# kocurvik/mdrp

Measured on AMD Instinct MI355X. Metric: image-pairs/sec (2000 corrs, 10k RANSAC iters), higher is better.
Workload: dtype f64

## Files before the change

### mdrp_amd/csrc/mdrp_capi.hip

```cpp
#include "../../include/mdrp.h"
#include "mdrp_kernels.h"
#include "mdrp_classic.h"
#include "mdrp_frontend.h"
#include "mdrp_schedule.h"
#include "mdrp_from_model.h"
#ifdef MDRP_SPLIT_TU
#define MDRP_INST extern
#include "mdrp_instances.h"
namespace mdrp {
MDRP_INSTANCES_FINAL_64
MDRP_INSTANCES_FINAL_256
MDRP_INSTANCES_CLASSIC
MDRP_INSTANCES_FROM_MODEL
}
#endif

#include <algorithm>
#include <cmath>
#include <cstdio>
#include <cstdlib>
#include <cstddef>
#include <cstring>
#include <functional>
#include <map>
// ... 483 lines not shown
        v.model_count = h->model_count[odd].as<int32_t>() + 2 * q; v.und_count = h->und_count.as<int32_t>() + 2 * q;
        v.surv1 = h->surv_count.as<int32_t>() + q; v.surv2 = h->surv2_count.as<int32_t>() + q;
        v.cand_stat = h->cand_stat.as<unsigned long long>() + 2 * q;
        v.rfrag = h->rfrag.as<uint4>() + q * groups_max * 64; v.trig = h->triggers.as<Trigger>() + q * trig_cap;
        return v;
    }

    int solve(const ChunkView &v, hipStream_t st_) {
        const RunParams &r = v.r;
        const int pc = v.pc;
        HIPCHK(hipMemsetAsync(v.model_count, 0, sizeof(int32_t) * 2 * pc, st_));
        if (v.c < 2 && presampled[v.c]) HIPCHK(hipStreamWaitEvent(st_, h->ev_sampled[v.c], 0));
        else samples(st_, r.chunk_len, v.samples);
        hipEvent_t v0, v1;
        if (int rc = get_events(h, &v0, &v1, 5)) return rc;
        HIPCHK(hipEventRecord(v0, st_));
        struct Stop { hipEvent_t e; hipStream_t s; ~Stop() { (void)hipEventRecord(e, s); } } stop_{v1, st_};
        if (classic) {
            const dim3 sgrid((r.chunk_len + 63) / 64, pc);
            if (kind == MDRP_SHARED_6PT)
                hipLaunchKernelGGL(kc_solve<CLASSIC_SHARED>, sgrid, dim3(64), 0, st_, r, v.st, v.samples, v.pts, v.models, v.slot_inl, v.tags, v.model_count);
            else if (kind == MDRP_RELPOSE_5PT) {
                const bool first_region = v.c == 0 && lay.n_chunks > 1;
                if (first_region && (size_t)sgrid.x > sz.red5_first_blocks) { g_err = "5-point first chunk longer than its Reduce5 region"; return MDRP_ERR_INVALID; }
                double *red5 = h->red5.as<double>() + ((first_region ? (size_t)batch * sz.red5_blocks : 0) + (size_t)v.p0 * sgrid.x) * RED5_STRIDE * 64;
                hipLaunchKernelGGL(kc_solve5_null, sgrid, dim3(64), SOLVE5N_LDS_BYTES, st_, r, v.st, v.samples, v.pts, red5);
                hipLaunchKernelGGL(kc_solve5_reduce, sgrid, dim3(64), SOLVE5_LDS_BYTES, st_, r, v.st, red5);
                hipLaunchKernelGGL(kc_solve5_roots, sgrid, dim3(64), SOLVE5B_LDS_BYTES, st_, r, v.st, v.samples, v.pts, red5, v.models, v.slot_inl, v.tags, v.model_count);
            }
            else
                hipLaunchKernelGGL(kc_solve<CLASSIC_FUND>, sgrid, dim3(64), SOLVE7_LDS_BYTES, st_, r, v.st, v.samples, v.pts, v.models, v.slot_inl, v.tags, v.model_count);
            return MDRP_OK;
        }
#define MDRP_SOLVE_LAUNCH(S)                                                                                                   \
    hipLaunchKernelGGL(k_solve<S>, dim3((r.chunk_len + solve_threads(S) - 1) / solve_threads(S), pc), dim3(solve_threads(S)), 0, st_, r, v.st, v.samples, v.pts, v.dep, v.models, v.slot_inl, v.tags, v.model_count, 0, r.chunk_len)
        switch (r.solver) {
        case SOLVER_P3P: MDRP_SOLVE_LAUNCH(SOLVER_P3P); break;
        case SOLVER_SHIFT: MDRP_SOLVE_LAUNCH(SOLVER_SHIFT); break;
        case SOLVER_SHARED: MDRP_SOLVE_LAUNCH(SOLVER_SHARED); break;
        default: MDRP_SOLVE_LAUNCH(SOLVER_VARYING); break;
        }
#undef MDRP_SOLVE_LAUNCH
        return MDRP_OK;
    }

    int count(const ChunkView &v) {
        unsigned long long *cstats = &cnt->progress.evals;
        hipEvent_t c0, c1;
        if (int rc = get_events(h, &c0, &c1, 1)) return rc;
        const bool two_phase = !v.first_of_run;
        uint32_t *tags_u = v.tags_sorted;
        int32_t *und_part = reinterpret_cast<int32_t *>(v.tags_sorted_other), *cplan = h->cplan.as<int32_t>();
        hipLaunchKernelGGL(k_count_plan, dim3(1), dim3(PLAN_THREADS), 0, s, v.pc, v.st, v.model_count, 2, CNT_WG_MODELS, cplan,
                           v.surv1, (const int32_t *)nullptr, two_phase ? v.und_count : (int32_t *)nullptr);
        const dim3 cgrid((unsigned)v.pc * (unsigned)((v.r.chunk_len * mps + CNT_WG_MODELS - 1) / CNT_WG_MODELS));
        HIPCHK(hipEventRecord(c0, s));
        MDRP_SWEEP_DISPATCH(k_count, kind, cgrid, dim3(CNT_THREADS), 0, s, v.r, v.st, v.rfrag, v.models,
                            v.tags, v.model_count, cplan, v.tags_v, v.surv1, cstats, (int32_t *)nullptr, (const int32_t *)nullptr,
                            1, tags_u, und_part, v.und_count, (const int32_t *)nullptr, v.cand_stat);
        if (two_phase) {
            hipLaunchKernelGGL(k_count_plan, dim3(1), dim3(PLAN_THREADS), 0, s, v.pc, v.st, v.und_count, 2, CNT_WG_MODELS, cplan,
                               (int32_t *)nullptr, (const int32_t *)nullptr, (int32_t *)nullptr);
            MDRP_SWEEP_DISPATCH(k_count, kind, cgrid, dim3(CNT_THREADS), 0, s, v.r, v.st, v.rfrag, v.models,
                                tags_u, v.und_count, cplan, v.tags_v, v.surv1, cstats, (int32_t *)nullptr, (const int32_t *)nullptr,
                                2, (uint32_t *)nullptr, (int32_t *)nullptr, (int32_t *)nullptr, und_part, v.cand_stat);
            h->count_launches++;
        }
        HIPCHK(hipEventRecord(c1, s));
        h->count_launches++;
        return MDRP_OK;
    }

    int bound(const ChunkView &v, Survivors &sv) {
        sv = Survivors{v.tags_v, v.surv1};
        if (!(use_bound && batch_call > 16 && !v.first_of_run)) return MDRP_OK;
        hipLaunchKernelGGL(k_count_plan, dim3(1), dim3(PLAN_THREADS), 0, s, v.pc, v.st, v.surv1, 1, BND_THREADS, h->cplan.as<int32_t>(), v.surv2, (const int32_t *)nullptr);
        const dim3 bgrid((unsigned)v.pc * (unsigned)((v.r.chunk_len * mps + BND_THREADS - 1) / BND_THREADS));
        unsigned long long *bstats = &cnt->progress.evals_bound;
        hipEvent_t b0, b1;
        if (int rc = get_events(h, &b0, &b1, 4)) return rc;
        HIPCHK(hipEventRecord(b0, s));
        MDRP_SWEEP_DISPATCH(k_bound, kind, bgrid, dim3(BND_THREADS), 0, s, v.r, v.st, v.pts, v.models, v.tags_v, v.surv1, h->cplan.as<int32_t>(), v.tags, v.surv2, bstats);
        HIPCHK(hipEventRecord(b1, s));
        sv = Survivors{v.tags, v.surv2};
        return MDRP_OK;
    }

    int score(const ChunkView &v, const Survivors &sv, hipEvent_t e0, hipEvent_t e1) {
        const bool wave = batch_call <= SCORE_WAVE_MAX_PAIRS, split = !wave && score_split && !v.first_of_run;
        const int models = v.r.chunk_len * mps;
        int32_t *plan = h->plan.as<int32_t>(), *totals = plan + 2 * (size_t)batch + 2;
        if (wave) hipLaunchKernelGGL(k_count_plan, dim3(1), dim3(PLAN_THREADS), 0, s, v.pc, v.st, sv.count, 1, SCW_THREADS / 64, plan, (int32_t *)nullptr, (const int32_t *)nullptr, (int32_t *)nullptr);
        hipLaunchKernelGGL(k_sort_tags, dim3(v.pc), dim3(256), 0, s, v.r, v.st, v.model_count, sv.count, sv.tags, v.tags_sorted);
        if (!wave) hipLaunchKernelGGL(k_plan, dim3(1), dim3(PLAN_THREADS), 0, s, v.pc, v.model_count, plan, totals, split ? SPLIT_HYP : SCORE_THREADS);
        HIPCHK(hipEventRecord(e0, s));
        const long long capped = (long long)h->num_cu * 32;
        if (wave) {
            const long long ub = (long long)v.pc * ((models + SCW_THREADS / 64 - 1) / (SCW_THREADS / 64));
            MDRP_SWEEP_DISPATCH(k_score_w, kind, dim3((unsigned)std::min(ub, capped)), dim3(SCW_THREADS), 0, s, v.r, v.st, v.pts, v.models, v.tags_sorted, v.model_count,
                                v.slot_score, v.slot_inl, plan);
        } else if (split) {
            const long long ub = (long long)v.pc * ((models + SPLIT_HYP - 1) / SPLIT_HYP + 1);
            MDRP_SWEEP_DISPATCH(k_score_split, kind, dim3((unsigned)std::min(ub, capped)), dim3(SPLIT_THREADS), 0, s, v.r, v.st, v.pts, v.models, v.tags_sorted, v.model_count,
                                v.slot_score, v.slot_inl, plan, totals);
        } else {
            const dim3 grid((unsigned)v.pc * (unsigned)((models + SCORE_THREADS - 1) / SCORE_THREADS));
            MDRP_SWEEP_DISPATCH(k_score, kind, grid, dim3(SCORE_THREADS), SCORE_TILE_BYTES, s, v.r, v.st, v.pts, v.models, v.tags_sorted, v.model_count,
                                v.slot_score, v.slot_inl, plan, totals);
        }
        HIPCHK(hipEventRecord(e1, s));
        h->sweep_launches++;
        return MDRP_OK;
    }

    void scan(const ChunkView &v) {
        unsigned long long *scan_stats = &cnt->progress.evals_sweep;
#define MDRP_SCAN(M, I) hipLaunchKernelGGL((k_scan<M, I>), dim3(v.pc), dim3(64), 0, s, v.r, v.st, v.slot_score, v.slot_inl, v.trig, trig_cap, v.model_count, scan_stats)
        if (mps == 16) MDRP_SCAN(16, 1);
// ... 1046 lines not shown
```

### mdrp_amd/csrc/mdrp_kernels.h

```cpp
#pragma once
#include <hip/hip_runtime.h>
#include <float.h>
#include "mdrp_logtab.h"
#include "mdrp_math.h"

#ifdef MDRP_SECONDARY_TU
#define MDRP_GLOBAL static __global__
#else
#define MDRP_GLOBAL __global__
#endif

namespace mdrp {

constexpr int PT_STRIDE = 6;
#define MDRP_TILE_PTS 512
#define MDRP_SCORE_MINWAVES 4
constexpr int TILE_PTS = MDRP_TILE_PTS;
constexpr size_t SCORE_TILE_BYTES = (size_t)TILE_PTS * (PT_STRIDE * sizeof(double) + 4 * sizeof(float));
#define MDRP_P1F_UNROLL 8
constexpr int PRUNE_EVERY = 4;
#define MDRP_DENSE_KEY 40
#define MDRP_SOLVE_MINWAVES 2
#define MDRP_SCORE_THREADS 256
constexpr int SCORE_THREADS = MDRP_SCORE_THREADS;
// ... 637 lines not shown
        const int mid = (lo + hi) >> 1;
        if (prefix[mid] <= w) lo = mid; else hi = mid;
    }
    return lo;
}

struct SweepItem { int pair; bool dense, live; uint32_t slot; size_t slot_base; };
__device__ __forceinline__ SweepItem sweep_item(const RunParams &rp, const int32_t *__restrict__ plan, const int32_t *__restrict__ model_count,
                                                const uint32_t *__restrict__ tags, int w, int per_wg, int idx) {
    SweepItem it;
    it.pair = plan_find(plan, rp.batch, w);
    const int blk_sparse = plan[rp.batch + 1 + it.pair];
    const int bi = w - plan[it.pair];
    it.dense = bi >= blk_sparse;
    const int i = (it.dense ? bi - blk_sparse : bi) * per_wg + idx;
    it.slot_base = (size_t)it.pair * rp.slot_stride;
    const int cnt_sparse = model_count[2 * it.pair], cnt_dense = model_count[2 * it.pair + 1];
    it.live = i < (it.dense ? cnt_dense : cnt_sparse);
    it.slot = it.live ? tags[it.slot_base + (it.dense ? rp.slot_stride - 1 - i : i)] : 0;
    return it;
}

#define MDRP_CNT_TILES 8
constexpr int CNT_TILES = MDRP_CNT_TILES;
constexpr int CNT_ROUNDS = (16 * CNT_TILES) / 64;
static_assert(CNT_TILES == 4 || CNT_TILES == 8, "a wavefront owns 64 or 128 hypotheses");
constexpr int CNT_WAVE_MODELS = 16 * CNT_TILES;
constexpr int CNT_THREADS = 256;
constexpr int CNT_WG_MODELS = CNT_WAVE_MODELS * (CNT_THREADS / 64);
typedef __bf16 bf16x8_t __attribute__((ext_vector_type(8)));
typedef float f32x4_t __attribute__((ext_vector_type(4)));

constexpr int PLAN_THREADS = 1024;
__device__ __forceinline__ int plan_block_scan(int v, int &total, int *s_w) {
    const int lane = threadIdx.x & 63, wave = threadIdx.x >> 6;
    int inc = v;
#pragma unroll
    for (int o = 1; o < 64; o <<= 1) { const int u = __shfl_up(inc, o, 64); if (lane >= o) inc += u; }
    __syncthreads();
    if (lane == 63) s_w[wave] = inc;
    __syncthreads();
    if (wave == 0) {
        const int x = lane < PLAN_THREADS / 64 ? s_w[lane] : 0;
        int xi = x;
#pragma unroll
        for (int o = 1; o < PLAN_THREADS / 64; o <<= 1) { const int u = __shfl_up(xi, o, 64); if (lane >= o) xi += u; }
        if (lane < PLAN_THREADS / 64) s_w[lane] = xi - x;
        if (lane == PLAN_THREADS / 64 - 1) s_w[PLAN_THREADS / 64] = xi;
    }
    __syncthreads();
    total = s_w[PLAN_THREADS / 64];
    return inc - v + s_w[wave];
}
MDRP_GLOBAL __launch_bounds__(PLAN_THREADS) void k_count_plan(int batch, const PairState *__restrict__ st, const int32_t *__restrict__ counts, int stride,
                                                             int per_wg, int32_t *__restrict__ plan, int32_t *__restrict__ zero_a,
                                                             const int32_t *__restrict__ begin = nullptr, int32_t *__restrict__ zero_b2 = nullptr ) {
    __shared__ int s_w[PLAN_THREADS / 64 + 1];
    int run = 0;
    for (int p0 = 0; p0 < batch; p0 += PLAN_THREADS) {
        const int p = p0 + threadIdx.x;
        const int b = (p < batch && st[p].active) ? (counts[stride * p] - (begin ? begin[stride * p] : 0) + per_wg - 1) / per_wg : 0;
        int tot;
        const int ex = plan_block_scan(b, tot, s_w);
        if (p < batch) { plan[p] = run + ex; if (zero_a) zero_a[p] = 0; if (zero_b2) zero_b2[2 * p] = 0; }
        run += tot;
    }
    if (threadIdx.x == 0) plan[batch] = run;
}

__device__ __forceinline__ int count_split_tiles(const PairState &ps, int n_tiles, const unsigned long long *__restrict__ cand_stat, int pair) {
    if (!(ps.best_min_score < DBL_MAX) || n_tiles < 4 || !cand_stat) return n_tiles;
    const unsigned long long cs = cand_stat[2 * pair], es = cand_stat[2 * pair + 1];
    if (es == 0) return n_tiles;
    const double rec_score = ps.best_min_score * (1.0 + 1e-12);
    long long bar = (long long)floor((double)ps.n - rec_score / ps.sq_thr);
    if (bar > (long long)ps.best_min_cnt) bar = (long long)ps.best_min_cnt;
    if (bar <= 0) return n_tiles;
    const double g = fmin(0.5, 1.1 * (double)cs / (double)es + 0.005);
    const long long ra = (long long)((double)((long long)ps.n - bar) / (1.0 - g)) + 32;
    const int ta = (int)((ra + 255) >> 8);
    return ta + 2 > n_tiles ? n_tiles : ta;
}

template <bool POSE, bool RAWF = false>
__global__ __launch_bounds__(CNT_THREADS, 4) void k_count(RunParams rp, const PairState *__restrict__ st, const uint4 *__restrict__ rfrag,
                                                          const Model *__restrict__ models, const uint32_t *__restrict__ tags,
                                                          const int32_t *__restrict__ model_count, const int32_t *__restrict__ plan,
                                                          uint32_t *__restrict__ tags_surv,
                                                          int32_t *__restrict__ surv_count, unsigned long long *__restrict__ stats,
                                                          int32_t *__restrict__ cand_out ,
                                                          const int32_t *__restrict__ tag_begin = nullptr ,
                                                          int phase = 0, uint32_t *__restrict__ tags_und = nullptr, int32_t *__restrict__ und_part = nullptr,
                                                          int32_t *__restrict__ und_count = nullptr, const int32_t *__restrict__ part_in = nullptr,
                                                          unsigned long long *__restrict__ cand_stat = nullptr ) {
    constexpr int A_TILE_GROUPS = 16;
    __shared__ uint4 s_lds[2 * A_TILE_GROUPS * 64];
    uint4 (*s_frag)[CNT_WAVE_MODELS][4] = reinterpret_cast<uint4 (*)[CNT_WAVE_MODELS][4]>(s_lds);
    static_assert(sizeof(uint4) * (CNT_THREADS / 64) * CNT_WAVE_MODELS * 4 <= sizeof(uint4) * 2 * A_TILE_GROUPS * 64, "fragment staging fits the tile buffers");
    const int total = plan[rp.batch];
    const int w = blockIdx.x;
    if (w >= total) return;
    const int pair = plan_find(plan, rp.batch, w);
    const int blk = w - plan[pair];
    const PairState &ps = st[pair];
    const int tbeg = tag_begin ? tag_begin[2 * pair] : 0;
    const int n = ps.n, cnt = model_count[2 * pair] - tbeg;
    const int tid = threadIdx.x, lane = tid & 63, wave = tid >> 6;
    const int m0 = blk * CNT_WG_MODELS + wave * CNT_WAVE_MODELS;
    const size_t slot_base = (size_t)pair * rp.slot_stride;
    const uint32_t *tags_p = tags + slot_base + tbeg;
    const double thr = ps.sq_thr;
    uint32_t slot_r[CNT_ROUNDS] = {};
    int part_r[CNT_ROUNDS] = {};
    Model mr[CNT_ROUNDS];
#pragma unroll
    for (int r = 0; r < CNT_ROUNDS; ++r) {
        const int i = m0 + 64 * r + lane;
        if (i < cnt) { slot_r[r] = tags_p[i] & 0xFFFFFFu; if (phase == 2) part_r[r] = part_in[slot_base + tbeg + i]; }
    }
#pragma unroll
    for (int r = 0; r < CNT_ROUNDS; ++r) {
        const Model *mp = models + slot_base + slot_r[r];
        const double2 *P = reinterpret_cast<const double2 *>(mp);
        const double2 q01 = P[0], q23 = P[1], t01 = P[2], t2s = P[3], f12 = P[5];
        mr[r].q[0] = q01.x; mr[r].q[1] = q01.y; mr[r].q[2] = q23.x; mr[r].q[3] = q23.y;
        mr[r].t[0] = t01.x; mr[r].t[1] = t01.y; mr[r].t[2] = t2s.x;
        mr[r].f1 = f12.x; mr[r].f2 = f12.y;
        mr[r].scale = t2s.y; mr[r].shift1 = RAWF ? P[4].x : 0.0;
    }
#pragma unroll
    for (int r = 0; r < CNT_ROUNDS; ++r) {
        const int i = m0 + 64 * r + lane;
        uint16_t eh[8], el[8], e8[3];
        float tb = 1.0f;
#pragma unroll
        for (int j = 0; j < 8; ++j) { eh[j] = 0; el[j] = 0; }
        e8[0] = e8[1] = e8[2] = 0;
        if (i < cnt) {
            double E[9];
            model_matrix<POSE, RAWF>(mr[r], E);
            count_setup_scaled(E, ps.box, thr, eh, el, e8, tb);
        }
        uint4 *dst = s_frag[wave][64 * r + lane];
        dst[0] = pack_bf16x8(eh);
        dst[1] = pack_bf16x8(el);
        dst[2] = make_uint4((uint32_t)e8[0] | ((uint32_t)e8[1] << 16), (uint32_t)e8[2], 0u, 0u);
        dst[3] = make_uint4(__float_as_uint(tb), 0u, 0u, 0u);
    }
    __syncthreads();
    const bool idle = m0 >= cnt;
    const int col = lane & 15, ksl = lane >> 4;
    const int part = ksl < 2 ? 0 : ksl - 1;
    bf16x8_t bfrag[CNT_TILES];
    float tbv[CNT_TILES];
    float cand[CNT_TILES];
#pragma unroll
    for (int t = 0; t < CNT_TILES; ++t) {
        const uint4 *src = s_frag[wave][16 * t + col];
        bfrag[t] = __builtin_bit_cast(bf16x8_t, src[part]);
        const float tb2 = __uint_as_float(src[3].x);
        tbv[t] = tb2;
        cand[t] = 0.f;
    }
    __syncthreads();
    f32x4_t acc[CNT_TILES];
    auto mfma2 = [&](const uint4 &araw, int t0) {
        const bf16x8_t a = __builtin_bit_cast(bf16x8_t, araw);
        asm volatile("v_mfma_f32_16x16x32_bf16 %0, %2, %3, 0\n\t"
                     "v_mfma_f32_16x16x32_bf16 %1, %2, %4, 0"
                     : "=&v"(acc[t0]), "=&v"(acc[t0 + 1]) : "v"(a), "v"(bfrag[t0]), "v"(bfrag[t0 + 1]));
    };
    auto test2 = [&](int t0) {
        float d0, d1, d2, d3, d4, d5, d6, d7;
        asm volatile("v_fma_f32 %2, -%10, %10, %18 clamp\n\t"
                     "v_fma_f32 %3, -%11, %11, %18 clamp\n\t"
                     "v_fma_f32 %4, -%12, %12, %18 clamp\n\t"
                     "v_fma_f32 %5, -%13, %13, %18 clamp\n\t"
                     "v_fma_f32 %6, -%14, %14, %19 clamp\n\t"
                     "v_fma_f32 %7, -%15, %15, %19 clamp\n\t"
                     "v_fma_f32 %8, -%16, %16, %19 clamp\n\t"
                     "v_fma_f32 %9, -%17, %17, %19 clamp\n\t"
                     "v_add_f32 %2, %2, %3\n\t"
                     "v_add_f32 %4, %4, %5\n\t"
                     "v_add_f32 %6, %6, %7\n\t"
                     "v_add_f32 %8, %8, %9\n\t"
                     "v_add_f32 %0, %0, %2\n\t"
                     "v_add_f32 %1, %1, %6\n\t"
                     "v_add_f32 %0, %0, %4\n\t"
                     "v_add_f32 %1, %1, %8"
                     : "+v"(cand[t0]), "+v"(cand[t0 + 1]), "=&v"(d0), "=&v"(d1), "=&v"(d2), "=&v"(d3), "=&v"(d4), "=&v"(d5), "=&v"(d6), "=&v"(d7)
                     : "v"(acc[t0][0]), "v"(acc[t0][1]), "v"(acc[t0][2]), "v"(acc[t0][3]), "v"(acc[t0 + 1][0]), "v"(acc[t0 + 1][1]),
                       "v"(acc[t0 + 1][2]), "v"(acc[t0 + 1][3]), "v"(tbv[t0]), "v"(tbv[t0 + 1]));
    };
    const int G = (n + 15) >> 4;
    const uint4 *A = rfrag + (size_t)pair * ((rp.n_max + 15) >> 4) * 64;
    const int n_tiles = (G + A_TILE_GROUPS - 1) / A_TILE_GROUPS;
    const int t_split = phase == 0 ? n_tiles : count_split_tiles(ps, n_tiles, cand_stat, pair);
    const int t_lo = phase == 2 ? t_split : 0, t_hi = phase == 1 ? t_split : n_tiles;
    uint4 stage[4];
    auto fetch = [&](int tile) {
        const int g0 = tile * A_TILE_GROUPS;
#pragma unroll
        for (int k = 0; k < 4; ++k) {
            const int idx = k * CNT_THREADS + tid;
            stage[k] = (g0 + (idx >> 6)) < G ? A[(size_t)g0 * 64 + idx] : make_uint4(0u, 0u, 0u, 0u);
        }
    };
    auto commit = [&](int buf) {
#pragma unroll
        for (int k = 0; k < 4; ++k) s_lds[buf * A_TILE_GROUPS * 64 + k * CNT_THREADS + tid] = stage[k];
    };
    if (t_lo >= t_hi) return;
    fetch(t_lo);
    commit(t_lo & 1);
    __syncthreads();
    for (int tile = t_lo; tile < t_hi; ++tile) {
        const int buf = tile & 1;
        if (tile + 1 < t_hi) fetch(tile + 1);
        if (!idle) {
            const uint4 *T = s_lds + buf * A_TILE_GROUPS * 64 + lane;
            uint4 f0 = T[0], f1 = T[64];
#pragma unroll
            for (int t = 0; t < CNT_TILES; t += 2) mfma2(f0, t);
#pragma unroll
            for (int g = 0; g < A_TILE_GROUPS; g += 2) {
                f0 = T[(size_t)min(g + 2, A_TILE_GROUPS - 1) * 64];
#pragma unroll
                for (int t = 0; t < CNT_TILES; t += 2) { test2(t); mfma2(f1, t); }
                f1 = T[(size_t)min(g + 3, A_TILE_GROUPS - 1) * 64];
                if (g + 2 < A_TILE_GROUPS) {
#pragma unroll
                    for (int t = 0; t < CNT_TILES; t += 2) { test2(t); mfma2(f0, t); }
                } else {
#pragma unroll
                    for (int t = 0; t < CNT_TILES; t += 2) test2(t);
                }
            }
        }
        if (tile + 1 < t_hi) commit(buf ^ 1);
        __syncthreads();
    }
    if (idle) return;
    uint32_t *s_out = reinterpret_cast<uint32_t *>(&s_frag[wave][0][0]);
    const int swept = (t_hi - t_lo) * A_TILE_GROUPS * 16, real = min(max(n - t_lo * A_TILE_GROUPS * 16, 0), swept);
    const int pad = swept - real;
    const bool split_a = phase == 1 && t_hi < n_tiles;
    const int rest = split_a ? n - t_hi * A_TILE_GROUPS * 16 : 0;
#pragma unroll
    for (int t = 0; t < CNT_TILES; ++t) {
        float o = cand[t];
        o += __shfl_xor(o, 16, 64);
        o += __shfl_xor(o, 32, 64);
        if (ksl == 0) s_out[16 * t + col] = (uint32_t)((int)o - pad);
    }
    __builtin_amdgcn_fence(__ATOMIC_RELEASE, "wavefront");
    __builtin_amdgcn_wave_barrier();
    const Bar bar(ps);
#pragma unroll
    for (int r = 0; r < CNT_ROUNDS; ++r) {
        const int i = m0 + 64 * r + lane;
        const bool live = i < cnt;
        const int cnd_here = live ? (int)s_out[64 * r + lane] + part_r[r] : 0;
        const int cnd = cnd_here + rest;
        if (cand_stat && phase == 1 && !split_a && bar.rec_cnt == 0 && !(ps.best_min_score < DBL_MAX)) {
            const int tot = wave_sum_i(cnd_here), lv = __popcll(__ballot(live));
            if (lane == 0 && lv) { atomicAdd(&cand_stat[2 * pair], (unsigned long long)tot); atomicAdd(&cand_stat[2 * pair + 1], (unsigned long long)lv * (unsigned long long)n); }
        }
        if (cand_out && live) cand_out[i] = cnd;
        const bool surv = live && ((long long)cnd > bar.rec_cnt || thr * (double)(n - cnd) < bar.rec_score);
        const unsigned long long ball = __ballot(surv);
        if (ball) {
            int base = 0;
            const int first = __ffsll((long long)ball) - 1;
            if (lane == first) base = atomicAdd(split_a ? &und_count[2 * pair] : &surv_count[pair], __popcll(ball));
            base = __shfl(base, first, 64);
            if (surv) {
                const size_t at = slot_base + base + __popcll(ball & ((1ull << lane) - 1ull));
                if (split_a) { tags_und[at] = slot_r[r]; und_part[at] = cnd_here; }
                else {
                    const uint32_t key = (uint32_t)min(PROBE_PTS, (int)(((long long)cnd * PROBE_PTS + n - 1) / n));
                    tags_surv[at] = slot_r[r] | (key << 24);
                }
            }
        }
    }
    if (stats && lane == 0 && wave == 0 && blk == 0) {
        if (phase != 2) atomicAdd(&stats[0], (unsigned long long)cnt * (unsigned long long)n);
        atomicAdd(&stats[1], (unsigned long long)(((cnt + 15) / 16) * 16) * (unsigned long long)swept);
    }
}

constexpr int BND_THREADS = 256;
#define MDRP_BND_TILE 256
constexpr int BND_TILE = MDRP_BND_TILE;

template <bool POSE, bool RAWF = false>
__global__ __launch_bounds__(BND_THREADS, 4) void k_bound(RunParams rp, const PairState *__restrict__ st, const double *__restrict__ pts,
                                                          const Model *__restrict__ models, const uint32_t *__restrict__ tags_in,
                                                          const int32_t *__restrict__ cnt_in, const int32_t *__restrict__ plan,
                                                          uint32_t *__restrict__ tags_out,
                                                          int32_t *__restrict__ cnt_out, unsigned long long *__restrict__ stats,
                                                          double *__restrict__ dbg_lb = nullptr ,
                                                          int32_t *__restrict__ dbg_cnt_ub = nullptr) {
    __shared__ float4 s_rec[BND_TILE];
    struct Open { uint32_t tag; int32_t sane; float Ef[9], eC, eD, thr_dn, c0, c1; double lb; };
    __shared__ Open s_open[BND_THREADS];
    __shared__ int s_wave_open[BND_THREADS / 64];
    const int total = plan[rp.batch];
    const int w = blockIdx.x;
    if (w >= total) return;
    const int pair = plan_find(plan, rp.batch, w);
    const int blk = w - plan[pair];
    const PairState &ps = st[pair];
    const int n = ps.n, cnt = cnt_in[pair];
    const int tid = threadIdx.x, lane = tid & 63, wave = tid >> 6;
    const int i = blk * BND_THREADS + tid;
    bool open = i < cnt;
    const size_t slot_base = (size_t)pair * rp.slot_stride;
    const double thr = ps.sq_thr;
    uint32_t tag = 0;
    float Ef[9], eC = 0.f, eD = 1.f, thr_dn = 0.f;
    bool sane = false;
#pragma unroll
    for (int q = 0; q < 9; ++q) Ef[q] = 0.f;
    if (open) {
        tag = tags_in[slot_base + i];
        const Model m = models[slot_base + (tag & 0xFFFFFFu)];
        double E[9];
        model_matrix<POSE, RAWF>(m, E);
        sane = bound_setup32(E, ps.box, thr, Ef, eC, eD, thr_dn);
    }
    double total_lb = 0.0;
    f32x2 cnt2 = {0.f, 0.f};
    const float thr_cnt = (float)(thr * (1.0 + 1e-5)) * (1.0f + 1e-6f);
    const float BIG = 1.2089258e24f;
    const f32x2 nbig = {-BIG, -BIG}, kcnt = {thr_cnt * BIG, thr_cnt * BIG};
    const Bar bar(ps);
    float4 *s_pair = s_rec;
    const double *gp = pts + (size_t)pair * rp.n_max * PT_STRIDE;
// ... 1369 lines not shown
```

### mdrp_amd/csrc/mdrp_math.h

```cpp
#pragma once
#include <math.h>
#include <stdint.h>

#if defined(__HIPCC__)
#define MDRP_HD __host__ __device__ __forceinline__
#else
#define MDRP_HD inline
#endif

namespace mdrp {

struct Model {
    double q[4];
    double t[3];
    double scale, shift1, shift2;
    double f1, f2;
};

MDRP_HD void model_identity(Model &m) {
    m.q[0] = 1.0; m.q[1] = 0.0; m.q[2] = 0.0; m.q[3] = 0.0;
    m.t[0] = 0.0; m.t[1] = 0.0; m.t[2] = 0.0;
    m.scale = 1.0; m.shift1 = 0.0; m.shift2 = 0.0; m.f1 = 1.0; m.f2 = 1.0;
}

// ... 739 lines not shown
    tb = (M < 1e30) ? (float)((T + 2e-6 * M) * (1.0 + 1e-6)) + 1e-30f : __builtin_inff();
    for (int i = 0; i < 9; ++i) Ef[i] = (float)E[i];
}

MDRP_HD bool filter_keeps(const float Ef[9], float tb, float a, float b, float c, float d) {
    const float e0 = fmaf(Ef[0], a, fmaf(Ef[1], b, Ef[2]));
    const float e1 = fmaf(Ef[3], a, fmaf(Ef[4], b, Ef[5]));
    const float e2 = fmaf(Ef[6], a, fmaf(Ef[7], b, Ef[8]));
    const float C = fmaf(c, e0, fmaf(d, e1, e2));
    return !(fabsf(C) > tb);
}

constexpr double COUNT_KAPPA = 6e-5;

MDRP_HD uint16_t bf16_bits(float x) {
    uint32_t u;
    __builtin_memcpy(&u, &x, 4);
    if ((u & 0x7fffffffu) > 0x7f800000u) return (uint16_t)((u >> 16) | 0x40u);
    u += 0x7fffu + ((u >> 16) & 1u);
    return (uint16_t)(u >> 16);
}
MDRP_HD float bf16_value(uint16_t b) {
    const uint32_t u = (uint32_t)b << 16;
    float f;
    __builtin_memcpy(&f, &u, 4);
    return f;
}
MDRP_HD void bf16_split(double x, uint16_t &h, uint16_t &l) {
    h = bf16_bits((float)x);
    l = bf16_bits((float)(x - (double)bf16_value(h)));
}
MDRP_HD void bf16_split3(double x, uint16_t &h, uint16_t &l, uint16_t &l2) {
    bf16_split(x, h, l);
    l2 = bf16_bits((float)(x - (double)bf16_value(h) - (double)bf16_value(l)));
}

MDRP_HD void count_monomials(double a, double b, double c, double d, double m[8]) {
    m[0] = a * c; m[1] = b * c; m[2] = c; m[3] = a * d; m[4] = b * d; m[5] = d; m[6] = a; m[7] = b;
}

MDRP_HD void count_setup(const double E[9], const double box[4], double thr, uint16_t eh[8], uint16_t el[8], uint16_t e8[3], float &tb) {
    const double ax = box[0], ay = box[1], cx = box[2], cy = box[3];
    const double e0 = fabs(E[0]) * ax + fabs(E[1]) * ay + fabs(E[2]), e1 = fabs(E[3]) * ax + fabs(E[4]) * ay + fabs(E[5]);
    const double g0 = fabs(E[0]) * cx + fabs(E[3]) * cy + fabs(E[6]), g1 = fabs(E[1]) * cx + fabs(E[4]) * cy + fabs(E[7]);
    const double dmax = (1.0 + 1e-9) * (e0 * e0 + e1 * e1 + g0 * g0 + g1 * g1);
    const double e2 = fabs(E[6]) * ax + fabs(E[7]) * ay + fabs(E[8]);
    const double M = e0 * cx + e1 * cy + e2;
    const double T = sqrt(thr * (1.0 + 1e-12) * dmax);
    tb = (M < 1e30) ? (float)((T + COUNT_KAPPA * M) * (1.0 + 1e-6)) + 1e-30f : __builtin_inff();
    for (int j = 0; j < 8; ++j) bf16_split(E[j], eh[j], el[j]);
    bf16_split3(E[8], e8[0], e8[1], e8[2]);
}

MDRP_HD void bf16_split_f32(float x, uint16_t &h, uint16_t &l) {
    h = bf16_bits(x);
    l = bf16_bits(x - bf16_value(h));
}
MDRP_HD void count_setup_scaled(const double E[9], const double box[4], double thr, uint16_t eh[8], uint16_t el[8], uint16_t e8[3], float &tb2) {
    const double ax = box[0], ay = box[1], cx = box[2], cy = box[3];
    const double e0 = fabs(E[0]) * ax + fabs(E[1]) * ay + fabs(E[2]), e1 = fabs(E[3]) * ax + fabs(E[4]) * ay + fabs(E[5]);
    const double g0 = fabs(E[0]) * cx + fabs(E[3]) * cy + fabs(E[6]), g1 = fabs(E[1]) * cx + fabs(E[4]) * cy + fabs(E[7]);
    const double dmax = (1.0 + 1e-9) * (e0 * e0 + e1 * e1 + g0 * g0 + g1 * g1);
    const double e2 = fabs(E[6]) * ax + fabs(E[7]) * ay + fabs(E[8]);
    const double M = e0 * cx + e1 * cy + e2;
    const float td = (float)(thr * (1.0 + 1e-12) * dmax), km = (float)(COUNT_KAPPA * M);
    const float tb = (sqrtf(td) + km) * (1.0f + 1e-6f) + 1e-30f;
    for (int j = 0; j < 8; ++j) { eh[j] = 0; el[j] = 0; }
    e8[0] = e8[1] = e8[2] = 0;
    tb2 = 1.0f;
    if (!(M < 1e30) || !(tb < 1e30f) || !(tb > 0.0f) || !(td > 1e-30f) || !(km > 1e-30f)) return;
    int ex;
    (void)frexpf(tb, &ex);
    const int k = 21 - ex;
    const double S = ldexp(1.0, k);
    for (int j = 0; j < 8; ++j) bf16_split_f32((float)(E[j] * S), eh[j], el[j]);
    const float c8 = (float)(E[8] * S);
    bf16_split_f32(c8, e8[0], e8[1]);
    e8[2] = bf16_bits((c8 - bf16_value(e8[0])) - bf16_value(e8[1]));
    const float tbs = ldexpf(tb, k);
    tb2 = (tbs * tbs) * (1.0f + 2e-7f);
}

constexpr double BOUND_SLACK = 2e-5;

MDRP_HD bool bound_setup32(const double E[9], const double box[4], double thr, float Ef[9], float &eC, float &eD, float &thr_dn) {
    const double ax = box[0], ay = box[1], cx = box[2], cy = box[3];
    const double e0 = fabs(E[0]) * ax + fabs(E[1]) * ay + fabs(E[2]), e1 = fabs(E[3]) * ax + fabs(E[4]) * ay + fabs(E[5]);
    const double g0 = fabs(E[0]) * cx + fabs(E[3]) * cy + fabs(E[6]), g1 = fabs(E[1]) * cx + fabs(E[4]) * cy + fabs(E[7]);
    const double dmax = e0 * e0 + e1 * e1 + g0 * g0 + g1 * g1;
    const double e2 = fabs(E[6]) * ax + fabs(E[7]) * ay + fabs(E[8]);
    const double M = e0 * cx + e1 * cy + e2;
    const bool sane = (M < 1e15) && (dmax < 1e30) && (dmax > 1e-30);
    eC = sane ? (float)(2e-6 * M * (1.0 + 1e-6)) + 1e-30f : 0.0f;
    eD = sane ? (float)(4e-6 * dmax * (1.0 + 1e-6)) + 1e-37f : 1.0f;
    float t = (float)thr;
    if ((double)t > thr && t > 0.0f) {
        uint32_t bits;
        __builtin_memcpy(&bits, &t, 4);
        --bits;
        __builtin_memcpy(&t, &bits, 4);
    }
    thr_dn = t;
    for (int i = 0; i < 9; ++i) Ef[i] = (float)E[i];
    return sane;
}

MDRP_HD float bound_r2_32(const float Ef[9], float eC, float eD, float a, float b, float c, float d) {
    const float e0 = fmaf(Ef[0], a, fmaf(Ef[1], b, Ef[2]));
    const float e1 = fmaf(Ef[3], a, fmaf(Ef[4], b, Ef[5]));
    const float e2 = fmaf(Ef[6], a, fmaf(Ef[7], b, Ef[8]));
    const float g0 = fmaf(Ef[0], c, fmaf(Ef[3], d, Ef[6]));
    const float g1 = fmaf(Ef[1], c, fmaf(Ef[4], d, Ef[7]));
    const float C = fmaf(c, e0, fmaf(d, e1, e2));
    const float den = fmaf(e0, e0, fmaf(e1, e1, fmaf(g0, g0, fmaf(g1, g1, eD))));
    const float t = fmaxf(fabsf(C) - eC, 0.0f);
#if defined(__HIP_DEVICE_COMPILE__)
    return (t * t) * __builtin_amdgcn_rcpf(den);
#else
    return (t * t) / den;
#endif
}

struct LmState {
    double R[9], t[3], s, u, v, f1, f2;
    double E[9], F[9];
    double if1, if2;
};

MDRP_HD void lm_state_from_model(const Model &m, bool focal, LmState &st) {
    quat_to_R(m.q, st.R);
    st.t[0] = m.t[0]; st.t[1] = m.t[1]; st.t[2] = m.t[2];
    st.s = m.scale; st.u = m.shift1; st.v = m.shift2;
    st.f1 = focal ? m.f1 : 1.0; st.f2 = focal ? m.f2 : 1.0;
// ... 255 lines not shown
```

Baseline: 129,400.

## Streamline count kernel epilogue, bf16 packing, and hoist split-tile planning

Moves the per-pair split-tile computation out of the count kernel and into the plan kernel, passing the result through und_count's odd slots. Replaces scalar bf16 splitting with packed two-element conversions and writes the fragments as whole words. Swaps the xor-shuffle reduction for permlane32/permlane16 swaps and batches the cand_stat atomics into one per wave. It also cuts register use by reloading tags and partials instead of keeping them in arrays, and uses 32-bit index arithmetic. The aim is to lower VGPR pressure and instruction count in the hot count kernel, at the cost of reusing und_count storage and adding some extra loads.

```diff
diff --git a/mdrp_amd/csrc/mdrp_capi.hip b/mdrp_amd/csrc/mdrp_capi.hip
--- a/mdrp_amd/csrc/mdrp_capi.hip
+++ b/mdrp_amd/csrc/mdrp_capi.hip
@@ -559,18 +559,19 @@
         uint32_t *tags_u = v.tags_sorted;
         int32_t *und_part = reinterpret_cast<int32_t *>(v.tags_sorted_other), *cplan = h->cplan.as<int32_t>();
         hipLaunchKernelGGL(k_count_plan, dim3(1), dim3(PLAN_THREADS), 0, s, v.pc, v.st, v.model_count, 2, CNT_WG_MODELS, cplan,
-                           v.surv1, (const int32_t *)nullptr, two_phase ? v.und_count : (int32_t *)nullptr);
+                           v.surv1, (const int32_t *)nullptr, two_phase ? v.und_count : (int32_t *)nullptr,
+                           v.cand_stat, v.und_count);
         const dim3 cgrid((unsigned)v.pc * (unsigned)((v.r.chunk_len * mps + CNT_WG_MODELS - 1) / CNT_WG_MODELS));
         HIPCHK(hipEventRecord(c0, s));
         MDRP_SWEEP_DISPATCH(k_count, kind, cgrid, dim3(CNT_THREADS), 0, s, v.r, v.st, v.rfrag, v.models,
                             v.tags, v.model_count, cplan, v.tags_v, v.surv1, cstats, (int32_t *)nullptr, (const int32_t *)nullptr,
-                            1, tags_u, und_part, v.und_count, (const int32_t *)nullptr, v.cand_stat);
+                            1, tags_u, und_part, v.und_count, (const int32_t *)nullptr, v.cand_stat, v.und_count);
         if (two_phase) {
             hipLaunchKernelGGL(k_count_plan, dim3(1), dim3(PLAN_THREADS), 0, s, v.pc, v.st, v.und_count, 2, CNT_WG_MODELS, cplan,
                                (int32_t *)nullptr, (const int32_t *)nullptr, (int32_t *)nullptr);
             MDRP_SWEEP_DISPATCH(k_count, kind, cgrid, dim3(CNT_THREADS), 0, s, v.r, v.st, v.rfrag, v.models,
                                 tags_u, v.und_count, cplan, v.tags_v, v.surv1, cstats, (int32_t *)nullptr, (const int32_t *)nullptr,
-                                2, (uint32_t *)nullptr, (int32_t *)nullptr, (int32_t *)nullptr, und_part, v.cand_stat);
+                                2, (uint32_t *)nullptr, (int32_t *)nullptr, (int32_t *)nullptr, und_part, (unsigned long long *)nullptr, v.und_count);
             h->count_launches++;
         }
         HIPCHK(hipEventRecord(c1, s));
diff --git a/mdrp_amd/csrc/mdrp_kernels.h b/mdrp_amd/csrc/mdrp_kernels.h
--- a/mdrp_amd/csrc/mdrp_kernels.h
+++ b/mdrp_amd/csrc/mdrp_kernels.h
@@ -713,22 +713,8 @@
     total = s_w[PLAN_THREADS / 64];
     return inc - v + s_w[wave];
 }
-MDRP_GLOBAL __launch_bounds__(PLAN_THREADS) void k_count_plan(int batch, const PairState *__restrict__ st, const int32_t *__restrict__ counts, int stride,
-                                                             int per_wg, int32_t *__restrict__ plan, int32_t *__restrict__ zero_a,
-                                                             const int32_t *__restrict__ begin = nullptr, int32_t *__restrict__ zero_b2 = nullptr ) {
-    __shared__ int s_w[PLAN_THREADS / 64 + 1];
-    int run = 0;
-    for (int p0 = 0; p0 < batch; p0 += PLAN_THREADS) {
-        const int p = p0 + threadIdx.x;
-        const int b = (p < batch && st[p].active) ? (counts[stride * p] - (begin ? begin[stride * p] : 0) + per_wg - 1) / per_wg : 0;
-        int tot;
-        const int ex = plan_block_scan(b, tot, s_w);
-        if (p < batch) { plan[p] = run + ex; if (zero_a) zero_a[p] = 0; if (zero_b2) zero_b2[2 * p] = 0; }
-        run += tot;
-    }
-    if (threadIdx.x == 0) plan[batch] = run;
-}
-
+constexpr int CNT_TILE_GROUPS = 16;
+__device__ __forceinline__ int count_tiles(int n) { return (((n + 15) >> 4) + CNT_TILE_GROUPS - 1) / CNT_TILE_GROUPS; }
 __device__ __forceinline__ int count_split_tiles(const PairState &ps, int n_tiles, const unsigned long long *__restrict__ cand_stat, int pair) {
     if (!(ps.best_min_score < DBL_MAX) || n_tiles < 4 || !cand_stat) return n_tiles;
     const unsigned long long cs = cand_stat[2 * pair], es = cand_stat[2 * pair + 1];
@@ -743,6 +729,30 @@
     return ta + 2 > n_tiles ? n_tiles : ta;
 }
 
+MDRP_GLOBAL __launch_bounds__(PLAN_THREADS) void k_count_plan(int batch, const PairState *__restrict__ st, const int32_t *__restrict__ counts, int stride,
+                                                             int per_wg, int32_t *__restrict__ plan, int32_t *__restrict__ zero_a,
+                                                             const int32_t *__restrict__ begin = nullptr, int32_t *__restrict__ zero_b2 = nullptr ,
+                                                             const unsigned long long *__restrict__ cand_stat = nullptr,
+                                                             int32_t *__restrict__ t_split = nullptr ) {
+    __shared__ int s_w[PLAN_THREADS / 64 + 1];
+    int run = 0;
+    for (int p0 = 0; p0 < batch; p0 += PLAN_THREADS) {
+        const int p = p0 + threadIdx.x;
+        const int b = (p < batch && st[p].active) ? (counts[stride * p] - (begin ? begin[stride * p] : 0) + per_wg - 1) / per_wg : 0;
+        int tot;
+        const int ex = plan_block_scan(b, tot, s_w);
+        if (p < batch) {
+            plan[p] = run + ex; if (zero_a) zero_a[p] = 0; if (zero_b2) zero_b2[2 * p] = 0;
+            if (t_split) t_split[2 * p + 1] = count_split_tiles(st[p], count_tiles(st[p].n), cand_stat, p);
+        }
+        run += tot;
+    }
+    if (threadIdx.x == 0) plan[batch] = run;
+}
+
+template <class T>
+__device__ __forceinline__ T &elem32(T *base, uint32_t idx) { return *(T *)((const char *)base + (idx * (uint32_t)sizeof(T))); }
+
 template <bool POSE, bool RAWF = false>
 __global__ __launch_bounds__(CNT_THREADS, 4) void k_count(RunParams rp, const PairState *__restrict__ st, const uint4 *__restrict__ rfrag,
                                                           const Model *__restrict__ models, const uint32_t *__restrict__ tags,
@@ -753,8 +763,9 @@
                                                           const int32_t *__restrict__ tag_begin = nullptr ,
                                                           int phase = 0, uint32_t *__restrict__ tags_und = nullptr, int32_t *__restrict__ und_part = nullptr,
                                                           int32_t *__restrict__ und_count = nullptr, const int32_t *__restrict__ part_in = nullptr,
-                                                          unsigned long long *__restrict__ cand_stat = nullptr ) {
-    constexpr int A_TILE_GROUPS = 16;
+                                                          unsigned long long *__restrict__ cand_stat = nullptr ,
+                                                          const int32_t *__restrict__ t_split_in = nullptr ) {
+    constexpr int A_TILE_GROUPS = CNT_TILE_GROUPS;
     __shared__ uint4 s_lds[2 * A_TILE_GROUPS * 64];
     uint4 (*s_frag)[CNT_WAVE_MODELS][4] = reinterpret_cast<uint4 (*)[CNT_WAVE_MODELS][4]>(s_lds);
     static_assert(sizeof(uint4) * (CNT_THREADS / 64) * CNT_WAVE_MODELS * 4 <= sizeof(uint4) * 2 * A_TILE_GROUPS * 64, "fragment staging fits the tile buffers");
@@ -766,18 +777,17 @@
     const PairState &ps = st[pair];
     const int tbeg = tag_begin ? tag_begin[2 * pair] : 0;
     const int n = ps.n, cnt = model_count[2 * pair] - tbeg;
-    const int tid = threadIdx.x, lane = tid & 63, wave = tid >> 6;
+    const int tid = threadIdx.x, lane = tid & 63, wave = __builtin_amdgcn_readfirstlane(tid >> 6);
     const int m0 = blk * CNT_WG_MODELS + wave * CNT_WAVE_MODELS;
     const size_t slot_base = (size_t)pair * rp.slot_stride;
     const uint32_t *tags_p = tags + slot_base + tbeg;
     const double thr = ps.sq_thr;
     uint32_t slot_r[CNT_ROUNDS] = {};
-    int part_r[CNT_ROUNDS] = {};
     Model mr[CNT_ROUNDS];
 #pragma unroll
     for (int r = 0; r < CNT_ROUNDS; ++r) {
         const int i = m0 + 64 * r + lane;
-        if (i < cnt) { slot_r[r] = tags_p[i] & 0xFFFFFFu; if (phase == 2) part_r[r] = part_in[slot_base + tbeg + i]; }
+        if (i < cnt) slot_r[r] = elem32(tags_p, (uint32_t)i) & 0xFFFFFFu;
     }
 #pragma unroll
     for (int r = 0; r < CNT_ROUNDS; ++r) {
@@ -792,20 +802,17 @@
 #pragma unroll
     for (int r = 0; r < CNT_ROUNDS; ++r) {
         const int i = m0 + 64 * r + lane;
-        uint16_t eh[8], el[8], e8[3];
+        uint32_t eh[4] = {0u, 0u, 0u, 0u}, el[4] = {0u, 0u, 0u, 0u}, e8[2] = {0u, 0u};
         float tb = 1.0f;
-#pragma unroll
-        for (int j = 0; j < 8; ++j) { eh[j] = 0; el[j] = 0; }
-        e8[0] = e8[1] = e8[2] = 0;
         if (i < cnt) {
             double E[9];
             model_matrix<POSE, RAWF>(mr[r], E);
-            count_setup_scaled(E, ps.box, thr, eh, el, e8, tb);
+            count_setup_words(E, ps.box, thr, eh, el, e8, tb);
         }
         uint4 *dst = s_frag[wave][64 * r + lane];
-        dst[0] = pack_bf16x8(eh);
-        dst[1] = pack_bf16x8(el);
-        dst[2] = make_uint4((uint32_t)e8[0] | ((uint32_t)e8[1] << 16), (uint32_t)e8[2], 0u, 0u);
+        dst[0] = make_uint4(eh[0], eh[1], eh[2], eh[3]);
+        dst[1] = make_uint4(el[0], el[1], el[2], el[3]);
+        dst[2] = make_uint4(e8[0], e8[1], 0u, 0u);
         dst[3] = make_uint4(__float_as_uint(tb), 0u, 0u, 0u);
     }
     __syncthreads();
@@ -856,7 +863,7 @@
     const int G = (n + 15) >> 4;
     const uint4 *A = rfrag + (size_t)pair * ((rp.n_max + 15) >> 4) * 64;
     const int n_tiles = (G + A_TILE_GROUPS - 1) / A_TILE_GROUPS;
-    const int t_split = phase == 0 ? n_tiles : count_split_tiles(ps, n_tiles, cand_stat, pair);
+    const int t_split = phase == 0 ? n_tiles : t_split_in[2 * pair + 1];
     const int t_lo = phase == 2 ? t_split : 0, t_hi = phase == 1 ? t_split : n_tiles;
     uint4 stage[4];
     auto fetch = [&](int tile) {
@@ -902,50 +909,65 @@
         __syncthreads();
     }
     if (idle) return;
+    int lane_e = lane;
+    asm volatile("" : "+v"(lane_e));
+    const int col_e = lane_e & 15, ksl_e = lane_e >> 4;
     uint32_t *s_out = reinterpret_cast<uint32_t *>(&s_frag[wave][0][0]);
     const int swept = (t_hi - t_lo) * A_TILE_GROUPS * 16, real = min(max(n - t_lo * A_TILE_GROUPS * 16, 0), swept);
     const int pad = swept - real;
     const bool split_a = phase == 1 && t_hi < n_tiles;
     const int rest = split_a ? n - t_hi * A_TILE_GROUPS * 16 : 0;
-#pragma unroll
-    for (int t = 0; t < CNT_TILES; ++t) {
-        float o = cand[t];
-        o += __shfl_xor(o, 16, 64);
-        o += __shfl_xor(o, 32, 64);
-        if (ksl == 0) s_out[16 * t + col] = (uint32_t)((int)o - pad);
+    {
+        const int tile0 = 2 * (ksl_e & 1) + (ksl_e >> 1);
+#pragma unroll
+        for (int h = 0; h < CNT_TILES / 4; ++h) {
+            float w[2];
+#pragma unroll
+            for (int i = 0; i < 2; ++i) {
+                const lme_u2 sw = __builtin_amdgcn_permlane32_swap(__float_as_uint(cand[4 * h + 2 * i]), __float_as_uint(cand[4 * h + 2 * i + 1]), false, false);
+                w[i] = __uint_as_float(sw.x) + __uint_as_float(sw.y);
+            }
+            const lme_u2 sw = __builtin_amdgcn_permlane16_swap(__float_as_uint(w[0]), __float_as_uint(w[1]), false, false);
+            const float x = __uint_as_float(sw.x) + __uint_as_float(sw.y);
+            s_out[16 * (4 * h + tile0) + col_e] = (uint32_t)((int)x - pad);
+        }
     }
     __builtin_amdgcn_fence(__ATOMIC_RELEASE, "wavefront");
     __builtin_amdgcn_wave_barrier();
     const Bar bar(ps);
+    const uint32_t un = (uint32_t)n;
+    int stat_c = 0;
 #pragma unroll
     for (int r = 0; r < CNT_ROUNDS; ++r) {
-        const int i = m0 + 64 * r + lane;
+        const int i = m0 + 64 * r + lane_e;
         const bool live = i < cnt;
-        const int cnd_here = live ? (int)s_out[64 * r + lane] + part_r[r] : 0;
+        const int cnd_here = live ? (int)s_out[64 * r + lane_e] + (phase == 2 ? elem32(part_in + slot_base + tbeg, (uint32_t)i) : 0) : 0;
         const int cnd = cnd_here + rest;
-        if (cand_stat && phase == 1 && !split_a && bar.rec_cnt == 0 && !(ps.best_min_score < DBL_MAX)) {
-            const int tot = wave_sum_i(cnd_here), lv = __popcll(__ballot(live));
-            if (lane == 0 && lv) { atomicAdd(&cand_stat[2 * pair], (unsigned long long)tot); atomicAdd(&cand_stat[2 * pair + 1], (unsigned long long)lv * (unsigned long long)n); }
-        }
-        if (cand_out && live) cand_out[i] = cnd;
+        stat_c += cnd_here;
+        if (cand_out && live) elem32(cand_out, (uint32_t)i) = cnd;
         const bool surv = live && ((long long)cnd > bar.rec_cnt || thr * (double)(n - cnd) < bar.rec_score);
         const unsigned long long ball = __ballot(surv);
         if (ball) {
             int base = 0;
             const int first = __ffsll((long long)ball) - 1;
-            if (lane == first) base = atomicAdd(split_a ? &und_count[2 * pair] : &surv_count[pair], __popcll(ball));
+            if (lane_e == first) base = atomicAdd(split_a ? &und_count[2 * pair] : &surv_count[pair], __popcll(ball));
             base = __shfl(base, first, 64);
             if (surv) {
-                const size_t at = slot_base + base + __popcll(ball & ((1ull << lane) - 1ull));
-                if (split_a) { tags_und[at] = slot_r[r]; und_part[at] = cnd_here; }
+                const uint32_t at = (uint32_t)(base + __popcll(ball & ((1ull << lane_e) - 1ull)));
+                const uint32_t slot = elem32(tags_p, (uint32_t)i) & 0xFFFFFFu;
+                if (split_a) { elem32(tags_und + slot_base, at) = slot; elem32(und_part + slot_base, at) = cnd_here; }
                 else {
-                    const uint32_t key = (uint32_t)min(PROBE_PTS, (int)(((long long)cnd * PROBE_PTS + n - 1) / n));
-                    tags_surv[at] = slot_r[r] | (key << 24);
+                    const uint32_t key = min((uint32_t)PROBE_PTS, ((uint32_t)cnd * (uint32_t)PROBE_PTS + un - 1u) / un);
+                    elem32(tags_surv + slot_base, at) = slot | (key << 24);
                 }
             }
         }
     }
-    if (stats && lane == 0 && wave == 0 && blk == 0) {
+    if (phase == 1 && cand_stat && !split_a && bar.rec_cnt == 0 && !(ps.best_min_score < DBL_MAX)) {
+        const int tot = __builtin_amdgcn_readfirstlane(wave_sum_i(stat_c)), lv = min(cnt - m0, CNT_WAVE_MODELS);
+        if (lane_e == 0) { atomicAdd(&cand_stat[2 * pair], (unsigned long long)tot); atomicAdd(&cand_stat[2 * pair + 1], (unsigned long long)lv * (unsigned long long)n); }
+    }
+    if (stats && lane_e == 0 && wave == 0 && blk == 0) {
         if (phase != 2) atomicAdd(&stats[0], (unsigned long long)cnt * (unsigned long long)n);
         atomicAdd(&stats[1], (unsigned long long)(((cnt + 15) / 16) * 16) * (unsigned long long)swept);
     }
diff --git a/mdrp_amd/csrc/mdrp_math.h b/mdrp_amd/csrc/mdrp_math.h
--- a/mdrp_amd/csrc/mdrp_math.h
+++ b/mdrp_amd/csrc/mdrp_math.h
@@ -815,11 +815,19 @@
     bf16_split3(E[8], e8[0], e8[1], e8[2]);
 }
 
-MDRP_HD void bf16_split_f32(float x, uint16_t &h, uint16_t &l) {
-    h = bf16_bits(x);
-    l = bf16_bits(x - bf16_value(h));
-}
-MDRP_HD void count_setup_scaled(const double E[9], const double box[4], double thr, uint16_t eh[8], uint16_t el[8], uint16_t e8[3], float &tb2) {
+MDRP_HD uint32_t bf16_pack2(float a, float b) {
+#if defined(__HIP_DEVICE_COMPILE__)
+    typedef float bf16_pack_f2 __attribute__((ext_vector_type(2)));
+    typedef __bf16 bf16_pack_b2 __attribute__((ext_vector_type(2)));
+    const bf16_pack_f2 v = {a, b};
+    return __builtin_bit_cast(uint32_t, __builtin_convertvector(v, bf16_pack_b2));
+#else
+    return (uint32_t)bf16_bits(a) | ((uint32_t)bf16_bits(b) << 16);
+#endif
+}
+MDRP_HD float bf16_pair_lo(uint32_t w) { return bf16_value((uint16_t)(w & 0xffffu)); }
+MDRP_HD float bf16_pair_hi(uint32_t w) { return bf16_value((uint16_t)(w >> 16)); }
+MDRP_HD void count_setup_words(const double E[9], const double box[4], double thr, uint32_t eh[4], uint32_t el[4], uint32_t e8[2], float &tb2) {
     const double ax = box[0], ay = box[1], cx = box[2], cy = box[3];
     const double e0 = fabs(E[0]) * ax + fabs(E[1]) * ay + fabs(E[2]), e1 = fabs(E[3]) * ax + fabs(E[4]) * ay + fabs(E[5]);
     const double g0 = fabs(E[0]) * cx + fabs(E[3]) * cy + fabs(E[6]), g1 = fabs(E[1]) * cx + fabs(E[4]) * cy + fabs(E[7]);
@@ -828,20 +836,37 @@
     const double M = e0 * cx + e1 * cy + e2;
     const float td = (float)(thr * (1.0 + 1e-12) * dmax), km = (float)(COUNT_KAPPA * M);
     const float tb = (sqrtf(td) + km) * (1.0f + 1e-6f) + 1e-30f;
-    for (int j = 0; j < 8; ++j) { eh[j] = 0; el[j] = 0; }
-    e8[0] = e8[1] = e8[2] = 0;
+    for (int j = 0; j < 4; ++j) { eh[j] = 0; el[j] = 0; }
+    e8[0] = e8[1] = 0;
     tb2 = 1.0f;
     if (!(M < 1e30) || !(tb < 1e30f) || !(tb > 0.0f) || !(td > 1e-30f) || !(km > 1e-30f)) return;
     int ex;
     (void)frexpf(tb, &ex);
     const int k = 21 - ex;
     const double S = ldexp(1.0, k);
-    for (int j = 0; j < 8; ++j) bf16_split_f32((float)(E[j] * S), eh[j], el[j]);
+    for (int j = 0; j < 4; ++j) {
+        const float a = (float)(E[2 * j] * S), b = (float)(E[2 * j + 1] * S);
+        const uint32_t h = bf16_pack2(a, b);
+        eh[j] = h;
+        el[j] = bf16_pack2(a - bf16_pair_lo(h), b - bf16_pair_hi(h));
+    }
     const float c8 = (float)(E[8] * S);
-    bf16_split_f32(c8, e8[0], e8[1]);
-    e8[2] = bf16_bits((c8 - bf16_value(e8[0])) - bf16_value(e8[1]));
+    const uint32_t h8 = bf16_pack2(c8, 0.0f);
+    const float r1 = c8 - bf16_pair_lo(h8);
+    const uint32_t l8 = bf16_pack2(r1, 0.0f);
+    e8[0] = h8 | (l8 << 16);
+    e8[1] = bf16_pack2(r1 - bf16_pair_lo(l8), 0.0f);
     const float tbs = ldexpf(tb, k);
     tb2 = (tbs * tbs) * (1.0f + 2e-7f);
+}
+MDRP_HD void count_setup_scaled(const double E[9], const double box[4], double thr, uint16_t eh[8], uint16_t el[8], uint16_t e8[3], float &tb2) {
+    uint32_t wh[4], wl[4], w8[2];
+    count_setup_words(E, box, thr, wh, wl, w8, tb2);
+    for (int j = 0; j < 4; ++j) {
+        eh[2 * j] = (uint16_t)(wh[j] & 0xffffu); eh[2 * j + 1] = (uint16_t)(wh[j] >> 16);
+        el[2 * j] = (uint16_t)(wl[j] & 0xffffu); el[2 * j + 1] = (uint16_t)(wl[j] >> 16);
+    }
+    e8[0] = (uint16_t)(w8[0] & 0xffffu); e8[1] = (uint16_t)(w8[0] >> 16); e8[2] = (uint16_t)(w8[1] & 0xffffu);
 }
 
 constexpr double BOUND_SLACK = 2e-5;
```

After: 130,500 (median of 6 runs). About the same (+0.9%).
